# greatscottgadgets/libbtbb

Measured on AMD Instinct MI355X. Metric: Gbit/s raw bitstream scanned (LAP_ANY, err<=2), higher is better.
Workload: dtype u64; 1 GPU; promiscuous LAP_ANY scan, 4 GiB packed single-channel synthetic bitstream per GPU, max_ac_errors=2, sync word every 4096 symbols; symbols_per_gpu=34359738305, hits_per_gpu=6402406, parallelism=time-sharded x1 (btbbx_shard_plan: slices + 63-symbol halo), no collectives

## Files before the change

libbtbb_amd/csrc/context.cpp:

```cpp
#include <stdarg.h>
#include <stdio.h>
#include <stdlib.h>
#include <string.h>
#include <mutex>
#include <shared_mutex>
#include <vector>
#include "common.h"

#define NO_DEVICE_SLOT BTBBX_MAX_DEVICES
static Ctx g_ctx[BTBBX_MAX_DEVICES + 1];
static std::mutex g_init_lock;
static std::shared_mutex g_tables_lock;

void ctx_scan_snapshot(ScanTables *tables, int *table_errors)
{
	std::shared_lock<std::shared_mutex> g(g_tables_lock);
	const Ctx &c = ctx();
	*tables = c.scan;
	*table_errors = c.table_errors;
}
static int g_table_errors = 0;
static thread_local char g_err[512] = "";

static int current_device()
// ... 402 lines not shown
#define BITMAP2_BITS_5 26
static int upload_tables(int max_ac_errors)
{
	const HostTables &t = host_tables();
	Ctx &c = ctx();

	uint64_t entries = 0, binom = 1;
	for (int k = 1; k <= max_ac_errors; k++) {
		binom = binom * (uint64_t)(58 - k + 1) / (uint64_t)k;
		entries += binom;
	}
	int bits = 12;
	while ((1ULL << bits) < 2 * entries + 16)
		bits++;
	while (bits < 20 && (1ULL << bits) < 16 * entries)
		bits++;
	MapBuilder mb;
	mb.slots.assign(1ULL << bits, HSLOT_EMPTY);
	mb.mask = (1ULL << bits) - 1;
	mb.shift = 32 - bits;
	if (max_ac_errors >= 3) {
		const int bits2 = max_ac_errors == 3 ? BITMAP2_BITS_3 : max_ac_errors == 4 ? BITMAP2_BITS_4 : BITMAP2_BITS_5;
		mb.shift2 = 32 - bits2;
		mb.bitmap2.assign(1u << (bits2 - 5), 0);
		mb.bitmap2[0] |= 1u;
	}
	int pos[5];
	for (int k = 1; k <= max_ac_errors; k++)
		mb.enumerate(t, 0, pos, 0, 0, k);

	std::vector<uint32_t> tabA(LDS_TABA_WORDS), tabB(LDS_TABB_WORDS);
	for (uint32_t v = 0; v < LDS_TABA_WORDS; v++) {
		uint64_t s = 0;
		for (int i = 0; i < TABA_BITS; i++)
			if ((v >> i) & 1)
				s ^= t.col[TABA_FIRST + i];
		tabA[v] = (uint32_t)s;
	}
	uint64_t kclass[2];
	kclass[0] = host_syndrome(((uint64_t)BARKER0 << 57) ^ SW_PN);
	kclass[1] = host_syndrome(((uint64_t)BARKER1 << 57) ^ SW_PN);
	for (uint32_t v = 0; v < (1u << TABB_BITS); v++) {
		uint64_t s = kclass[0];
		for (int i = 0; i < TABB_BITS; i++)
			if ((v >> i) & 1)
				s ^= t.col[TABA_FIRST + TABA_BITS + i];
		tabB[v] = (uint32_t)s;
	}

	std::vector<uint32_t> slide_bitmap(SLIDE_WORDS, 0u);
	if (max_ac_errors <= 2) {
		const int rc_slide = build_slide_set(t, max_ac_errors, slide_bitmap);
		if (rc_slide < 0)
			return rc_slide;
		if (slide_bitmap[0] & 3u) {
			set_error("btbbx_init: internal: index 0 / 1 of the sliding checks is a member of the candidate set");
			return BTBBX_E_ARG;
		}
	}

	std::vector<uint32_t> slide4, slide4b;
	if (max_ac_errors == 3 || max_ac_errors == 4) {
		const int rc4 = build_two_level_sets(t, max_ac_errors, slide4, slide4b);
		if (rc4 < 0)
			return rc4;
	} else if (max_ac_errors == 5) {
		const int rc5 = build_five_error_front_set(t, slide4b);
		if (rc5 < 0)
			return rc5;
	}

	size_t off_a = 0, off_b = off_a + 4 * LDS_TABA_WORDS, off_m = off_b + 4 * LDS_TABB_WORDS;
	size_t off_s = off_m;
	size_t off_s4 = off_s + 4 * SLIDE_WORDS, off_s4b = off_s4 + 4 * slide4.size();
	size_t total = off_s4b + 4 * slide4b.size();
	struct Fresh {
		void *tab = nullptr, *hslots = nullptr, *bitmap2 = nullptr;
		~Fresh() { if (tab) (void)hipFree(tab); if (hslots) (void)hipFree(hslots); if (bitmap2) (void)hipFree(bitmap2); }
	} fresh;
	if (!mb.bitmap2.empty()) {
		HIP_TRY(hipMalloc(&fresh.bitmap2, mb.bitmap2.size() * 4));
		HIP_TRY(hipMemcpy(fresh.bitmap2, mb.bitmap2.data(), mb.bitmap2.size() * 4, hipMemcpyHostToDevice));
	}
	HIP_TRY(hipMalloc(&fresh.tab, total));
	HIP_TRY(hipMalloc(&fresh.hslots, mb.slots.size() * sizeof(uint64_t)));
	char *base = (char *)fresh.tab;
	HIP_TRY(hipMemcpy(base + off_a, tabA.data(), 4 * LDS_TABA_WORDS, hipMemcpyHostToDevice));
	HIP_TRY(hipMemcpy(base + off_b, tabB.data(), 4 * LDS_TABB_WORDS, hipMemcpyHostToDevice));
	HIP_TRY(hipMemcpy(base + off_s, slide_bitmap.data(), 4 * SLIDE_WORDS, hipMemcpyHostToDevice));
	if (!slide4.empty())
		HIP_TRY(hipMemcpy(base + off_s4, slide4.data(), 4 * slide4.size(), hipMemcpyHostToDevice));
	if (!slide4b.empty())
		HIP_TRY(hipMemcpy(base + off_s4b, slide4b.data(), 4 * slide4b.size(), hipMemcpyHostToDevice));
	HIP_TRY(hipMemcpy(fresh.hslots, mb.slots.data(), mb.slots.size() * sizeof(uint64_t), hipMemcpyHostToDevice));
	HIP_TRY(hipDeviceSynchronize());
	std::unique_lock<std::shared_mutex> swap_guard(g_tables_lock);
	if (c.d_retired_tab) (void)hipFree(c.d_retired_tab);
	if (c.d_retired_hslots) (void)hipFree(c.d_retired_hslots);
	if (c.d_retired_bitmap2) (void)hipFree(c.d_retired_bitmap2);
	c.d_retired_tab = c.d_tab_block;
	c.d_retired_hslots = c.d_hslots;
	c.d_retired_bitmap2 = c.d_bitmap2;
	c.d_tab_block = fresh.tab;
	c.d_hslots = fresh.hslots;
	c.d_bitmap2 = fresh.bitmap2;
	fresh.tab = fresh.hslots = fresh.bitmap2 = nullptr;
	base = (char *)c.d_tab_block;
	c.scan.tabA = (const uint32_t *)(base + off_a);
	c.scan.tabB = (const uint32_t *)(base + off_b);
	c.scan.slide_bitmap = (const uint32_t *)(base + off_s);
	c.scan.slide4_bitmap = slide4.empty() ? nullptr : (const uint32_t *)(base + off_s4);
	c.scan.slide4b_bitmap = slide4b.empty() ? nullptr : (const uint32_t *)(base + off_s4b);
	c.scan.hslots = (const uint64_t *)c.d_hslots;
	c.scan.hmask = mb.mask;
	c.scan.kclass[0] = kclass[0];
	c.scan.kclass[1] = kclass[1];
	c.scan.kdiff = (uint32_t)(kclass[0] ^ kclass[1]);
	c.scan.hi_mask[0] = c.scan.hi_mask[1] = 0;
	for (int j = 0; j < 57; j++) {
		if ((t.col[j] >> 32) & 1) c.scan.hi_mask[0] |= 1ULL << j;
		if ((t.col[j] >> 33) & 1) c.scan.hi_mask[1] |= 1ULL << j;
	}
	c.scan.bitmap2 = (const uint32_t *)c.d_bitmap2;
	c.scan.bitmap2_shift = (uint32_t)mb.shift2;
	c.table_errors = max_ac_errors;
	return BTBBX_OK;
}

static int init_current_device(int max_ac_errors)
{
	const int dev = current_device();
	if (dev == NO_DEVICE_SLOT) {
		int d = -1;
		(void)hipGetDevice(&d);
		set_error("btbbx_init: HIP device ordinal %d is not below BTBBX_MAX_DEVICES = %d (or hipGetDevice failed)", d,
			  BTBBX_MAX_DEVICES);
		return BTBBX_E_ARG;
	}
	Ctx &c = g_ctx[dev];
	if (g_table_errors == 0 && max_ac_errors > 0)
		g_table_errors = max_ac_errors;
	if (!c.ready) {
		int n = 0;
		hipError_t e = hipGetDeviceCount(&n);
		if (e != hipSuccess || n <= 0) {
			set_error("btbbx_init: no HIP device available (%s) -- this library has no CPU path",
				  e == hipSuccess ? "device count 0" : hipGetErrorString(e));
			return BTBBX_E_NODEVICE;
		}
		c.device = dev;
		hipDeviceProp_t prop;
		HIP_TRY(hipGetDeviceProperties(&prop, dev));
		c.num_cus = prop.multiProcessorCount > 0 ? prop.multiProcessorCount : 256;
		int rc = chain_upload(host_tables());
		if (rc)
			return rc;
		rc = upload_tables(g_table_errors);
		if (rc)
			return rc;
		c.ready = true;
		return BTBBX_OK;
	}
	if (c.table_errors != g_table_errors)
		return upload_tables(g_table_errors);
	return BTBBX_OK;
}
// ... 116 lines not shown
```

libbtbb_amd/csrc/scan_core.h:

```cpp
#pragma once
#include "tile_scan.h"

#define FULL_MASK 0xffffffffffffffffULL

struct ScanArgs {
	const uint64_t *words;
	uint64_t n_words;
	uint64_t pitch_words;
	uint64_t search_bits;
	uint64_t tiles_per_stream;
	uint64_t n_tiles;
	uint32_t xcd_tiles;
	uint32_t ring_margin;
	uint32_t full_tiles;
	uint32_t n_streams;
	uint32_t msb;
	uint32_t lap;
	uint64_t syncword;
	int max_err;
	btbbx_hit *hits;
	uint32_t hit_cap;
	uint32_t *hit_count;
	unsigned long long *first;
	uint32_t *bucket_cnt;
// ... 23 lines not shown
#define PROF_MARK(k) do { (void)(k); } while (0)
#define PROF_PIN(x) do { } while (0)
#endif

__device__ __forceinline__ void count_bucket(const ScanArgs &a, uint32_t stream, uint64_t offset)
{
	if (a.bucket_cnt)
		atomicAdd(&a.bucket_cnt[((uint64_t)stream * a.bucket_mul + offset) >> a.bucket_shift], 1u);
}

__device__ __forceinline__ void emit_hit(const ScanArgs &a, uint32_t stream, uint64_t offset,
					 uint32_t lap, uint32_t nerr)
{
	if (a.first) {
		unsigned long long v = ((unsigned long long)offset << 32) | ((unsigned long long)(lap & 0xffffff) << 8) | nerr;
		atomicMin(a.first, v);
		return;
	}
	uint32_t idx = atomicAdd(a.hit_count, 1u);
	if (idx < a.hit_cap) {
		btbbx_hit h;
		h.offset = offset;
		h.lap = lap;
		h.ac_errors = (uint8_t)nerr;
		h.reserved = 0;
		h.stream = (uint16_t)stream;
		a.hits[idx] = h;
		count_bucket(a, stream, offset);
	}
}

__device__ __forceinline__ uint64_t stream_ld(const uint64_t *p)
{
	return *p;
}
__device__ __forceinline__ uint32_t msb_dword(uint32_t x)
{
	return __builtin_bswap32(__brev(x));
}
__device__ __forceinline__ uint64_t load_word(const uint64_t *base, uint64_t j, uint64_t n_words)
{
	return j < n_words ? stream_ld(base + j) : 0ULL;
}

typedef __attribute__((address_space(3))) uint32_t lds_u32_t;
__device__ __forceinline__ uint32_t lds_ld(uint32_t byte_off) { return *reinterpret_cast<lds_u32_t *>(byte_off); }
__device__ __forceinline__ void lds_st(uint32_t byte_off, uint32_t v) { *reinterpret_cast<lds_u32_t *>(byte_off) = v; }
typedef __attribute__((address_space(3))) uint16_t lds_u16_t;
__device__ __forceinline__ uint32_t lds_ld16(uint32_t byte_off) { return *reinterpret_cast<lds_u16_t *>(byte_off); }
__device__ __forceinline__ uint64_t sign16_after_shl(uint32_t x, uint32_t sh)
{
	uint32_t r;
	uint64_t m;
	asm("v_lshlrev_b16 %1, %2, %3\n\tv_cmp_gt_i16_e64 %0, 0, %1" : "=s"(m), "=&v"(r) : "v"(sh), "v"(x));
	return m;
}
typedef __attribute__((address_space(3))) u32x4 lds_u32x4_t;
__device__ __forceinline__ u32x4 lds_ld4(uint32_t byte_off) { return *reinterpret_cast<lds_u32x4_t *>(byte_off); }
__device__ __forceinline__ void lds_st4(uint32_t byte_off, u32x4 v) { *reinterpret_cast<lds_u32x4_t *>(byte_off) = v; }
__device__ __forceinline__ void lds_st_rec(uint32_t byte_off, u32x4 v)
{
	lds_st(byte_off, v.x);
	lds_st(byte_off + 4u, v.y);
	lds_st(byte_off + 8u, v.z);
	lds_st(byte_off + 12u, v.w);
}
__device__ __forceinline__ void lds_st_rec2(uint32_t byte_off, uint32_t x, uint32_t y, uint32_t z, uint32_t w)
{
	asm volatile("ds_write2_b32 %0, %1, %2 offset1:1\n\tds_write2_b32 %0, %3, %4 offset0:2 offset1:3"
		     : : "v"(byte_off), "v"(x), "v"(y), "v"(z), "v"(w) : "memory");
}

#define SYN3_WORDS 640u
#define SYN3_BYTES (4u * SYN3_WORDS)
static_assert(TABA_FIRST == 34 && TABA_BITS == 11 && TABB_BITS == 12, "the SYN3 tables are cut for window bits 34 .. 56 as 8 + 8 + 7");
__device__ __forceinline__ uint32_t syn3_entry(const ScanTables &t, uint32_t i)
{
	if (i < 256u)
		return t.tabA[i];
	if (i < 512u)
		return t.tabA[((i - 256u) & 7u) << 8] ^ t.tabB[(i - 256u) >> 3] ^ t.tabB[0];
	return t.tabB[(i - 512u) << 5];
}
template <bool LDS_TABLES = true, bool TWO = false>
__device__ __forceinline__ bool verify_lap_any(const ScanArgs &a, uint64_t w, uint32_t &lap, uint32_t &nerr_out, uint32_t syn3_off = 0)
{
	uint32_t win = (uint32_t)(w >> 57);
	uint32_t cls = __popc(win ^ BARKER1) <= 1 ? 1u : 0u;
	uint64_t sw = (w & LOW57) | ((uint64_t)(cls ? BARKER1 : BARKER0) << 57);
	const uint64_t low = w & LOW57;
	const uint32_t ia = (uint32_t)(low >> TABA_FIRST) & ((1u << TABA_BITS) - 1), ib = (uint32_t)(low >> (TABA_FIRST + TABA_BITS));
	uint32_t s_lo;
	if constexpr (TWO) {
		const uint32_t hi = (uint32_t)(low >> 32);
		s_lo = (uint32_t)low ^ lds_ld(syn3_off + (hi & 0x3fcu)) ^ lds_ld(syn3_off + 1024u + ((hi >> 8) & 0x3fcu))
		       ^ lds_ld(syn3_off + 2048u + ((hi >> 16) & 0x1fcu)) ^ (cls ? a.t.kdiff : 0u);
	} else {
		s_lo = (uint32_t)low ^ (LDS_TABLES ? lds_ld(LDS_OFF_TABA + (ia << 2)) : a.t.tabA[ia])
		       ^ (LDS_TABLES ? lds_ld(LDS_OFF_TABB + (ib << 2)) : a.t.tabB[ib]) ^ (cls ? a.t.kdiff : 0u);
	}
	uint32_t s_hi;
	if constexpr (TWO) {
		const uint32_t l0 = (uint32_t)low, l1 = (uint32_t)(low >> 32);
		const uint32_t f0 = (l0 & (uint32_t)a.t.hi_mask[0]) ^ (l1 & (uint32_t)(a.t.hi_mask[0] >> 32));
		const uint32_t f1 = (l0 & (uint32_t)a.t.hi_mask[1]) ^ (l1 & (uint32_t)(a.t.hi_mask[1] >> 32));
		s_hi = ((uint32_t)(a.t.kclass[cls] >> 32) ^ (__popc(f0) & 1) ^ ((__popc(f1) & 1) << 1)) & 3;
	} else {
		s_hi = ((uint32_t)(a.t.kclass[cls] >> 32) ^ (__popcll(low & a.t.hi_mask[0]) & 1)
			^ ((__popcll(low & a.t.hi_mask[1]) & 1) << 1)) & 3;
	}
	const uint64_t syn = ((uint64_t)s_hi << 32) | s_lo;
	if (!TWO && a.t.bitmap2) {
		const uint32_t i2 = (s_lo * 0x9E3779B1u) >> a.t.bitmap2_shift;
		if (!((a.t.bitmap2[i2 >> 5] >> (i2 & 31)) & 1))
			return false;
	}
	uint32_t nerr = 0;
	if (syn) {
		uint64_t h = ((((uint32_t)syn ^ (uint32_t)(syn >> 32)) * 0x9E3779B1u) >> (32 - __popcll(a.t.hmask))) & a.t.hmask;
		for (;;) {
			uint64_t slot = a.t.hslots[h];
			if (slot == HSLOT_EMPTY)
				return false;
			if ((slot & 0x3ffffffffULL) == syn) {
				if constexpr (TWO) {
					const uint32_t p0 = (uint32_t)(slot >> 34) & 63, p1 = (uint32_t)(slot >> 40) & 63;
					sw ^= (1ULL << p0) | (1ULL << p1);
					nerr = p1 != 63 ? 2u : 1u;
					break;
				}
				uint64_t err = 0;
#pragma unroll
				for (int i = 0; i < 5; i++) {
					uint32_t pos = (uint32_t)(slot >> (34 + 6 * i)) & 63;
					if (pos != 63)
						err |= 1ULL << pos;
				}
				sw ^= err;
				nerr = __popcll(err);
				break;
			}
			h = (h + 1) & a.t.hmask;
		}
	}
	lap = (uint32_t)(sw >> 34) & 0xffffff;
	nerr_out = nerr;
	return (int)nerr <= a.max_err;
}


__device__ __forceinline__ void barker32(uint32_t dm, uint32_t dh, uint32_t valid, uint32_t &pass, uint32_t &cls)
{
	const uint32_t s0 = alignbit(dh, dm, 25), s1 = alignbit(dh, dm, 26), s2 = alignbit(dh, dm, 27);
	const uint32_t s3 = alignbit(dh, dm, 28), s4 = alignbit(dh, dm, 29), s5 = alignbit(dh, dm, 30);
	const uint32_t s6 = alignbit(dh, dm, 31);
	const uint32_t a = BITOP3(s0, s1, s2, 0x69);
	const uint32_t ca = BITOP3(s0, s1, s2, 0x17);
	const uint32_t b = BITOP3(s3, s4, s5, 0x69);
	const uint32_t cb = BITOP3(s3, s4, s5, 0xd4);
	const uint32_t cc = BITOP3(a, b, s6, 0xe8);
	pass = BITOP3(ca, cb, cc, 0x81) & valid;
	cls = BITOP3(ca, cb, cc, 0x01);
}

struct Probe { uint32_t x, offA, offB; };

__device__ __forceinline__ Probe probe_addr(uint32_t e0, uint32_t e1, uint32_t e2, uint32_t cls,
					    uint32_t kdiff, uint32_t p)
{
	Probe r;
	const uint32_t wlo = alignbit(e1, e0, p);
	const uint32_t whi = alignbit(e2, e1, p);
	r.offA = whi & (((1u << TABA_BITS) - 1) << 2);
	r.offB = (whi >> (TABA_FIRST - 32 + TABA_BITS - 2)) & (((1u << TABB_BITS) - 1) << 2);
	const uint32_t cmask = (uint32_t)__builtin_amdgcn_sbfe(cls, p, 1);
	r.x = BITOP3(cmask, kdiff, wlo, 0x6a);
	return r;
}

#ifndef PRIO_FILTER
#define PRIO_FILTER 0
#define PRIO_LOOP 2
#define PRIO_CAND 3
#endif
struct SlideTapList { int n; int k[32]; };
template <uint64_t TAPS>
constexpr SlideTapList slide_tap_list()
{
	SlideTapList l = {0, {0}};
	for (int k = 0; k < 64; k++)
		if ((TAPS >> k) & 1)
			l.k[l.n++] = k;
	return l;
}
template <uint64_t TAPS>
__device__ __forceinline__ uint32_t slide32(uint32_t e0, uint32_t e1, uint32_t e2)
{
	constexpr SlideTapList taps = slide_tap_list<TAPS>();
	uint32_t plane[32];
#pragma unroll
	for (int i = 0; i < taps.n; i++) {
		const int k = taps.k[i];
		if (k == 0)
			plane[i] = e0;
		else if (k < 32)
			plane[i] = alignbit(e1, e0, k);
		else if (k == 32)
			plane[i] = e1;
		else
			plane[i] = alignbit(e2, e1, k - 32);
	}
	uint32_t acc = plane[0];
#pragma unroll
	for (int i = 1; i + 1 < taps.n; i += 2)
		acc = xor3(acc, plane[i], plane[i + 1]);
	if ((taps.n & 1) == 0)
		acc ^= plane[taps.n - 1];
	return acc;
}


#define TILE_ORDER(a, first_tile, tile_step, n_mine) \
	uint32_t first_tile = blockIdx.x, tile_step = gridDim.x, n_mine; \
	if (a.xcd_tiles) { \
		const uint32_t xcd = blockIdx.x & 7, lo_t = xcd * a.xcd_tiles; \
		const uint32_t hi_t = min((uint64_t)lo_t + a.xcd_tiles, a.n_tiles); \
		tile_step = gridDim.x >> 3; \
		first_tile = lo_t + (blockIdx.x >> 3); \
		n_mine = first_tile < hi_t ? (hi_t - first_tile + tile_step - 1) / tile_step : 0; \
	} else { \
// ... 63 lines not shown
```

libbtbb_amd/csrc/scan_slide.h:

```cpp
#pragma once
#include "scan_core.h"

#define SLIDE_TILES 2
#define SLIDE4_TILES 3
#define SLIDE_WGS 2
#define SLIDE_THREADS 768
#define SLIDE_FIXED 6
#define SLIDE_DRAIN_AT 60u
#define SLIDE_DRAIN_AT_ORD 40u
struct SlideStd {
	static constexpr int BITS = SLIDE_BITS, THREADS = SLIDE_THREADS, WGS = SLIDE_WGS;
	static constexpr uint64_t TAPS = SLIDE_TAPS, TAPS_B = 0;
	static constexpr bool LEVEL2 = false, INVERT = false, DENSE = false;
	static constexpr bool TWO_ERRORS = true;
};
struct Slide4 {
	static constexpr int BITS = SLIDE4_BITS, THREADS = 1024, WGS = 1;
	static constexpr uint64_t TAPS = SLIDE4_TAPS, TAPS_B = SLIDE4B_TAPS;
	static constexpr bool LEVEL2 = true, INVERT = true, DENSE = true;
	static constexpr bool TWO_ERRORS = false;
};
template <class CFG> struct SlideGeom {
	static constexpr uint32_t SET_WORDS = 1u << (CFG::BITS - 5), SET_BYTES = 4u * SET_WORDS;
	static constexpr uint32_t WAVES_PER_EU = CFG::WGS * CFG::THREADS / 256;
#ifdef SCAN_PROFILE
	static constexpr uint32_t RING = 64;
#else
	static constexpr uint32_t RING = CFG::WGS == 2 ? 64 : 128;
#endif
	static constexpr uint32_t LANE_WORDS = 63;
	static constexpr uint32_t TILE_WORDS = CFG::THREADS / 64 * LANE_WORDS;
	static constexpr uint32_t RING_END = SET_BYTES + CAND_BYTES * (CFG::THREADS / 64) * RING;
	static constexpr uint32_t SYN3_OFF = RING_END;
	static constexpr uint32_t PROF_OFF = SYN3_OFF + (CFG::TWO_ERRORS ? SYN3_BYTES : 0u);
#ifdef SCAN_PROFILE
	static constexpr uint32_t LDS_BYTES = PROF_OFF + 128u * (CFG::THREADS / 64);
#else
	static constexpr uint32_t LDS_BYTES = PROF_OFF;
#endif
	static_assert((uint64_t)LDS_BYTES * CFG::WGS <= 160u * 1024u, "the workgroups a CU is cut for must fit its 160 KiB of LDS");
};

template <class CFG, int TILES, bool MSB, bool ORD = false>
__global__ __launch_bounds__(CFG::THREADS) __attribute__((amdgpu_waves_per_eu(SlideGeom<CFG>::WAVES_PER_EU, SlideGeom<CFG>::WAVES_PER_EU)))
void scan_slide_kernel(ScanArgs a)
{
	extern __shared__ uint32_t lds[];
	if (a.gate && *a.gate == 0)
		return;
	constexpr uint32_t RING = SlideGeom<CFG>::RING;
	constexpr bool ABS = !CFG::LEVEL2;
	constexpr uint32_t THREADS = CFG::THREADS, SET_WORDS = SlideGeom<CFG>::SET_WORDS, SET_BYTES = SlideGeom<CFG>::SET_BYTES;

	const uint32_t tid = threadIdx.x;
	const uint32_t lane = tid & 63;
	const uint32_t wave = __builtin_amdgcn_readfirstlane(tid >> 6);
	constexpr uint32_t LANE_WORDS = SlideGeom<CFG>::LANE_WORDS, TILE_WORDS = SlideGeom<CFG>::TILE_WORDS;
	const uint32_t wid = wave * LANE_WORDS + lane;
	uint32_t live = lane != 63 ? 0xffffffffu : 0u;
	asm volatile("" : "+v"(live));
	const uint32_t ring_off = SET_BYTES + CAND_BYTES * wave * RING;

	TILE_ORDER(a, first_tile, tile_step, n_mine)

	{
		const uint4 *src = reinterpret_cast<const uint4 *>(CFG::LEVEL2 ? a.t.slide4_bitmap : a.t.slide_bitmap);
		uint4 *dst = reinterpret_cast<uint4 *>(lds);
		auto rev16 = [](uint32_t x) { const uint32_t r = __brev(x); return (r >> 16) | (r << 16); };
		for (uint32_t i = tid; i < SET_WORDS / 4; i += THREADS) {
			const uint4 v = src[i];
			dst[i] = make_uint4(rev16(v.x), rev16(v.y), rev16(v.z), rev16(v.w));
		}
	}
	constexpr uint32_t SYN3_OFF = SlideGeom<CFG>::SYN3_OFF;
	if constexpr (CFG::TWO_ERRORS) {
		for (uint32_t i = tid; i < SYN3_WORDS; i += THREADS)
			lds_st(SYN3_OFF + 4u * i, syn3_entry(a.t, i));
	}
	__syncthreads();

#ifdef SCAN_PROFILE
	const uint32_t prof_off = SlideGeom<CFG>::PROF_OFF + 128u * wave;
	if (lane < 32)
		lds_st(prof_off + 4u * lane, 0u);
	uint64_t prof_t;
	asm volatile("s_memtime %0\n\ts_waitcnt lgkmcnt(0)" : "=s"(prof_t) : : "memory");
#endif
	uint32_t q_head = 0, q_tail = 0;
	uint32_t code_tile = 0;
	CODE_WORD_CLOSURE(TILE_WORDS, LANE_WORDS, code_tile = t);
	HIT_QUEUE_CLOSURES();
	auto drain = [&](uint32_t n) {
		bool hit = false;
		uint32_t stream = 0, lap = 0, nerr = 0;
		uint64_t offset = 0;
		u32x4 rec = {0u, 0u, 0u, 0u};
		if (lane < n)
			rec = lds_ld4(ring_off + CAND_BYTES * ((q_head + lane) & (RING - 1)));
		const uint32_t code = rec.x;
		const uint64_t word = code_word(code, stream);
		if (lane < n) {
			const uint64_t w = ((uint64_t)alignbit(rec.w, rec.z, code) << 32) | alignbit(rec.z, rec.y, code);
			offset = word * 64 + (code & 63);
			hit = verify_lap_any<false, CFG::TWO_ERRORS>(a, w, lap, nerr, SYN3_OFF);
		}
		if constexpr (ORD) {
			const uint64_t hm = __ballot(hit);
			if (hm) {
				uint32_t rank = 0, count = 0;
				const uint32_t it_mine = code >> 12;
				const uint32_t it_lo = (uint32_t)__builtin_amdgcn_readfirstlane((int)it_mine) & ~1u;
				const uint32_t it_hi = (uint32_t)__builtin_amdgcn_readlane((int)it_mine, (int)(n - 1)) | 1u;
				bool fast = it_hi - it_lo < 64u;
				if (fast) {
					const uint32_t key = (it_mine - it_lo) & 63u;
					lds_st(ring_off + 4u * lane, 0u);
					uint32_t idx = 0;
					if (hit) {
						idx = __hip_atomic_fetch_add(reinterpret_cast<lds_u32_t *>(ring_off + 4u * key), 1u, __ATOMIC_RELAXED, __HIP_MEMORY_SCOPE_WORKGROUP);
						if (idx < 4u)
							*reinterpret_cast<__attribute__((address_space(3))) uint16_t *>(ring_off + 256u + 8u * key + 2u * idx) = (uint16_t)(code & 0xfffu);
					}
					asm volatile("s_waitcnt lgkmcnt(0)" ::: "memory");
					if (hit)
						count = lds_ld(ring_off + 4u * key);
					if (__ballot(count > 4u)) {
						fast = false;
					} else if (hit) {
						const uint32_t lo2 = lds_ld(ring_off + 256u + 8u * key), hi2 = lds_ld(ring_off + 260u + 8u * key);
						const uint32_t mine = code & 0xfffu;
						rank = ((lo2 & 0xffffu) < mine ? 1u : 0u);
						rank += count > 1u && (lo2 >> 16) < mine ? 1u : 0u;
						rank += count > 2u && (hi2 & 0xffffu) < mine ? 1u : 0u;
						rank += count > 3u && (hi2 >> 16) < mine ? 1u : 0u;
					}
				}
				if (!fast) {
					rank = count = 0;
					for (uint64_t r = hm; r; r &= r - 1) {
						const uint32_t cj = (uint32_t)__builtin_amdgcn_readlane((int)code, (int)__builtin_ctzll(r));
						const bool same = (code ^ cj) < 4096u;
						count += same ? 1u : 0u;
						rank += same && cj < code ? 1u : 0u;
					}
				}
				const uint32_t seg = stream * a.segs_per_stream + code_tile * (THREADS / 64) + wave;
				uint4 out;
				out.x = (uint32_t)offset;
				out.y = (uint32_t)(offset >> 32);
				out.z = lap;
				out.w = nerr | (stream << 16);
				const bool spill = hit && rank >= a.seg_slot_n;
				if (hit && !spill)
					a.seg_slots[(uint64_t)seg * a.seg_slot_n + rank] = (uint64_t)(code & 0xfffu) | ((uint64_t)lap << 12) | ((uint64_t)nerr << 36);
				if (hit && rank + 1 == count)
					a.seg_cnt[seg] = (uint16_t)count;
				const uint64_t om = __ballot(spill);
				if (om) {
					uint32_t base = 0;
					if (lane == 0)
						base = atomicAdd(a.ovf_count, (uint32_t)__popcll(om));
					base = __builtin_amdgcn_readfirstlane(base);
					const uint32_t idx = base + __builtin_amdgcn_mbcnt_hi((uint32_t)(om >> 32), __builtin_amdgcn_mbcnt_lo((uint32_t)om, 0));
					if (spill) {
						if (idx < a.ovf_cap) {
							reinterpret_cast<uint4 *>(a.ovf_recs)[idx] = out;
							a.ovf_meta[idx] = make_uint2(seg, rank);
						} else {
							*a.irregular = 1u;
						}
					}
				}
			}
		} else {
			push_hits(hit, stream, offset, lap, nerr);
		}
		q_head += n;
	};

	struct Cursor { uint32_t stream; uint32_t t; const uint64_t *tp; };
	const uint32_t tiles_per_stream = (uint32_t)a.tiles_per_stream;
	Cursor cur = {a.n_streams, 0, a.words};
	uint32_t handed = 0;
	auto tile_address = [&](const Cursor &c) { return a.words + (uint64_t)c.stream * a.pitch_words + (uint64_t)c.t * TILE_WORDS; };
	if (n_mine) {
		cur.stream = a.n_streams > 1 ? first_tile / tiles_per_stream : 0;
		cur.t = first_tile - cur.stream * tiles_per_stream;
		cur.tp = tile_address(cur);
	}
	auto step_words = [&]() {
		uint32_t ts = tile_step;
		asm volatile("" : "+s"(ts));
		return (uint64_t)ts * TILE_WORDS;
	};
	auto advance = [&](Cursor &c) {
		if (++handed >= n_mine) {
			c.stream = a.n_streams;
			return;
		}
		c.t += tile_step;
		c.tp += step_words();
		if (c.t >= tiles_per_stream) {
			while (c.t >= tiles_per_stream && c.stream < a.n_streams) {
				c.t -= tiles_per_stream;
				c.stream++;
			}
			c.tp = tile_address(c);
		}
	};
	auto tile_full = [&](uint32_t tt) { return tt < a.full_tiles; };
	uint32_t voff = wid * 8u;
	asm volatile("" : "+v"(voff));
	auto load_pair = [&](const Cursor &c, uint64_t &lo, uint64_t &hi) {
		uint32_t bytes = 0;
		if (c.stream < a.n_streams) {
			bytes = (TILE_WORDS + 2u) * 8u;
			if (!tile_full(c.t)) {
				const uint64_t first = (uint64_t)c.t * TILE_WORDS;
				const uint64_t left = first < a.n_words ? a.n_words - first : 0;
				bytes = (uint32_t)(left < TILE_WORDS + 2u ? left : TILE_WORDS + 2u) * 8u;
			}
		}
		const __amdgpu_buffer_rsrc_t rsrc = __builtin_amdgcn_make_buffer_rsrc(const_cast<uint64_t *>(c.tp), 0, (int)bytes, 0x00020000);
		const u32x4 v = __builtin_amdgcn_raw_buffer_load_b128(rsrc, (int)voff, 0, 0);
		lo = ((uint64_t)v.y << 32) | v.x;
		hi = ((uint64_t)v.w << 32) | v.z;
	};

	Cursor tc[TILES];
	uint64_t lo[TILES], hi[TILES];
#pragma unroll
	for (int u = 0; u < TILES; u++) {
		tc[u] = cur;
		load_pair(cur, lo[u], hi[u]);
		advance(cur);
	}

	for (uint32_t it = 0; tc[0].stream < a.n_streams; it += TILES) {
		__builtin_amdgcn_s_setprio(PRIO_FILTER);
		uint32_t d[TILES][4], m[TILES][2], c[TILES][3];
		uint32_t c2[TILES][CFG::LEVEL2 ? 3 : 1];
#pragma unroll
		for (int u = 0; u < TILES; u++) {
			d[u][0] = (uint32_t)lo[u]; d[u][1] = (uint32_t)(lo[u] >> 32);
			d[u][2] = (uint32_t)hi[u]; d[u][3] = (uint32_t)(hi[u] >> 32);
			if constexpr (MSB) {
#pragma unroll
				for (int k = 0; k < 4; k++)
					d[u][k] = msb_dword(d[u][k]);
			}
			uint32_t cls_unused;
			barker32(d[u][1], d[u][2], live, m[u][0], cls_unused);
			barker32(d[u][2], d[u][3], live, m[u][1], cls_unused);
			if (tc[u].stream >= a.n_streams) {
				m[u][0] = m[u][1] = 0;
			} else if (!tile_full(tc[u].t)) {
				const uint64_t first_off = ((uint64_t)tc[u].t * TILE_WORDS + wid) * 64;
				const uint64_t valid = first_off >= a.search_bits ? 0ULL
					: (a.search_bits - first_off >= 64 ? FULL_MASK : ((1ULL << (a.search_bits - first_off)) - 1));
				m[u][0] &= (uint32_t)valid;
				m[u][1] &= (uint32_t)(valid >> 32);
			}
			c[u][0] = slide32<CFG::TAPS>(d[u][0], d[u][1], d[u][2]);
			c[u][1] = slide32<CFG::TAPS>(d[u][1], d[u][2], d[u][3]);
			if constexpr (CFG::INVERT) {
				c[u][0] = ~c[u][0];
				c[u][1] = ~c[u][1];
			}
			c[u][2] = (uint32_t)__builtin_amdgcn_ds_bpermute((int)((lane + 1) << 2), (int)c[u][0]);
			if constexpr (CFG::LEVEL2) {
				c2[u][0] = slide32<CFG::TAPS_B>(d[u][0], d[u][1], d[u][2]);
				c2[u][1] = slide32<CFG::TAPS_B>(d[u][1], d[u][2], d[u][3]);
				c2[u][2] = (uint32_t)__builtin_amdgcn_ds_bpermute((int)((lane + 1) << 2), (int)c2[u][0]);
			}
		}

		uint64_t C[TILES][2];
#pragma unroll
		for (int u = 0; u < TILES; u++)
#pragma unroll
			for (int h = 0; h < 2; h++)
				C[u][h] = ((uint64_t)(ABS ? c[u][h + 1] : (c[u][h + 1] | 0x80000000u)) << 32) | c[u][h];
		struct Stage { uint32_t v[TILES][2], bw[TILES][2]; };
		auto any_left = [&]() {
			uint32_t any = 0;
#pragma unroll
			for (int u = 0; u < TILES; u++)
				any |= m[u][0] | m[u][1];
			return __ballot(any != 0) != 0;
		};
		uint32_t pos2[TILES][2];
		auto event_chain = [&](int u, int h, uint64_t cm) {
			const bool cand = __builtin_amdgcn_inverse_ballot_w64(cm);
			const uint32_t room = RING - (q_tail - q_head);
			uint32_t in_wave;
			asm("s_bcnt1_i32_b64 %0, %1" : "=s"(in_wave) : "s"(cm) : "scc");
			const uint32_t n = min(in_wave, room);
			if (cand) {
				uint32_t lane6 = lane << 6;
				asm volatile("" : "+v"(lane6));
				uint32_t pos;
				if constexpr (ABS)
					pos = pos2[u][h];
				else if constexpr (CFG::LEVEL2)
					pos = pos2[u][h];
				else
					asm("v_ffbh_u32 %0, %1" : "=v"(pos) : "v"((uint32_t)(C[u][h] >> 32)));
				const uint32_t code = pos | lane6 | (((it + u) << 12) | (h << 5));
				const u32x4 rec = {code, d[u][h], d[u][h + 1], d[u][h + 2]};
				if (in_wave == 1 && room) {
					lds_st_rec(ring_off + CAND_BYTES * (q_tail & (RING - 1)), rec);
				} else {
					const uint32_t rank = __builtin_amdgcn_mbcnt_hi((uint32_t)(cm >> 32),
							__builtin_amdgcn_mbcnt_lo((uint32_t)cm, 0));
					if (rank < room) {
						lds_st_rec(ring_off + CAND_BYTES * ((q_tail + rank) & (RING - 1)), rec);
					} else {
						uint32_t stream, lap, nerr, cold = code;
						asm volatile("" : "+v"(cold));
						const uint64_t word = code_word(cold, stream);
						const uint32_t wlo = alignbit(rec.z, rec.y, pos), whi = alignbit(rec.w, rec.z, pos);
// ... 132 lines not shown
		auto level2_take = [&]() {
			if (!any_sent)
				return;
			uint64_t cms[TILES][2], any = 0;
#pragma unroll
			for (int u = 0; u < TILES; u++)
#pragma unroll
				for (int h = 0; h < 2; h++) {
					cms[u][h] = sent[u][h] & __ballot((int32_t)(w2[u][h] << (v2[u][h] & 31)) < 0);
					any |= cms[u][h];
				}
			any_sent = 0;
			if (any)
				events(cms);
		};
		auto pass = [&]() {
			Stage g;
#pragma unroll
			for (int u = 0; u < TILES; u++)
#pragma unroll
				for (int h = 0; h < 2; h++)
					step(u, h, g);
			__builtin_amdgcn_sched_barrier(0);
			uint64_t cms[TILES][2], any = 0;
#pragma unroll
			for (int u = 0; u < TILES; u++)
#pragma unroll
				for (int h = 0; h < 2; h++) {
					cms[u][h] = member(u, h, g);
					any |= cms[u][h];
				}
			if constexpr (CFG::LEVEL2) {
				level2_take();
				static_assert(!CFG::LEVEL2 || TILES == 3, "the scalar OR below is written for six chains");
				uint64_t any2;
				asm("s_or_b64 %0, %1, %2\n\ts_or_b64 %0, %0, %3\n\ts_or_b64 %0, %0, %4\n\ts_or_b64 %0, %0, %5\n\ts_or_b64 %0, %0, %6"
				    : "=&s"(any2) : "s"(cms[0][0]), "s"(cms[0][1]), "s"(cms[1][0]), "s"(cms[1][1]), "s"(cms[TILES - 1][0]), "s"(cms[TILES - 1][1]) : "scc");
				if (any2)
					level2_send(cms);
			} else if (any) {
				note_events(cms);
			}
		};
		auto sparse_tail = [&]() {
			uint64_t live[TILES][2], anyl = 0;

#pragma unroll
			for (int u = 0; u < TILES; u++)
#pragma unroll
				for (int h = 0; h < 2; h++) {
					live[u][h] = __ballot(m[u][h] != 0);
					anyl |= live[u][h];
				}
			while (anyl) {
				Stage g;
				uint64_t cms[TILES][2], anyc = 0;
				anyl = 0;
#pragma unroll
				for (int u = 0; u < TILES; u++)
#pragma unroll
					for (int h = 0; h < 2; h++) {
						cms[u][h] = 0;
						if (!live[u][h])
							continue;
						step(u, h, g);
						cms[u][h] = member(u, h, g);
						anyc |= cms[u][h];
						live[u][h] = __ballot(m[u][h] != 0);
						anyl |= live[u][h];
					}
				if (anyc)
					note_events(cms);
			}
		};
#ifdef SCAN_PROFILE
#pragma unroll
		for (int u = 0; u < TILES; u++) {
			PROF_PIN(m[u][0]); PROF_PIN(m[u][1]); PROF_PIN(c[u][0]); PROF_PIN(c[u][1]); PROF_PIN(c[u][2]);
		}
#endif
		PROF_MARK(0);
		uint32_t pass_no = 1;
		if constexpr (!CFG::DENSE) {
			__builtin_amdgcn_s_setprio(PRIO_LOOP);
#pragma unroll 1
			for (int k = 0; k < SLIDE_FIXED; k++) {
				pass();
				PROF_MARK(pass_no < 13 ? pass_no : 13);
				pass_no++;
			}
			sparse_tail();
			append_noted();
			PROF_MARK(pass_no < 13 ? pass_no : 13);
			__builtin_amdgcn_s_setprio(PRIO_CAND);
			PROF_MARK(16);
			if (q_tail - q_head >= (RING == 64 ? (ORD ? SLIDE_DRAIN_AT_ORD : SLIDE_DRAIN_AT) : 64u))
				drain(q_tail - q_head > 64 ? 64 : q_tail - q_head);
		} else {
			for (;;) {
				__builtin_amdgcn_s_setprio(PRIO_LOOP);
				bool more = true;
				while (q_tail - q_head + a.ring_margin <= RING) {
					if (!any_left()) {
						more = false;
						break;
					}
					pass();
					PROF_MARK(pass_no < 13 ? pass_no : 13);
					pass_no++;
				}
				if constexpr (CFG::LEVEL2)
					level2_take();
				__builtin_amdgcn_s_setprio(PRIO_CAND);
				PROF_MARK(16);
				if (more || q_tail - q_head >= 32u)
					drain(q_tail - q_head > 64 ? 64 : q_tail - q_head);
				if (!more)
					break;
			}
		}
		(void)pass_no;
		PROF_MARK(18);
#pragma unroll
		for (int u = 0; u < TILES; u++) {
			tc[u] = cur;
			load_pair(cur, lo[u], hi[u]);
			advance(cur);
		}
		PROF_MARK(19);
	}
	while (q_tail != q_head)
		drain(q_tail - q_head > 64 ? 64 : q_tail - q_head);
	flush_hits();
#ifdef SCAN_PROFILE
	if (lane < 32)
		atomicAdd(&g_scan_prof[lane], (unsigned long long)lds_ld(prof_off + 4u * lane));
#endif
}
```

Baseline: 13290 Gbit/s.

## Split slide drain into issue and deferred verify to hide hash-slot latency

The sparse slide path's candidate drain is split in two. The first half computes syndromes and issues the global hash-slot load, fetching two adjacent slots as one vector load. The second half finishes probing and pushes hits at the top of the next tile iteration, so the global load latency overlaps with tile loads and filtering. A duplicated sentinel slot is appended to the table so the paired load stays in bounds. The cost is extra live registers across the loop and added code-path complexity.

```diff
diff --git a/libbtbb_amd/csrc/context.cpp b/libbtbb_amd/csrc/context.cpp
--- a/libbtbb_amd/csrc/context.cpp
+++ b/libbtbb_amd/csrc/context.cpp
@@ -508,6 +508,7 @@
 		HIP_TRY(hipMalloc(&fresh.bitmap2, mb.bitmap2.size() * 4));
 		HIP_TRY(hipMemcpy(fresh.bitmap2, mb.bitmap2.data(), mb.bitmap2.size() * 4, hipMemcpyHostToDevice));
 	}
+	mb.slots.push_back(mb.slots[0]);
 	HIP_TRY(hipMalloc(&fresh.tab, total));
 	HIP_TRY(hipMalloc(&fresh.hslots, mb.slots.size() * sizeof(uint64_t)));
 	char *base = (char *)fresh.tab;
diff --git a/libbtbb_amd/csrc/scan_core.h b/libbtbb_amd/csrc/scan_core.h
--- a/libbtbb_amd/csrc/scan_core.h
+++ b/libbtbb_amd/csrc/scan_core.h
@@ -129,70 +129,104 @@
 		return t.tabA[((i - 256u) & 7u) << 8] ^ t.tabB[(i - 256u) >> 3] ^ t.tabB[0];
 	return t.tabB[(i - 512u) << 5];
 }
+__device__ __forceinline__ uint64_t lap_syndrome2(const ScanArgs &a, uint64_t w, uint64_t &sw, uint32_t syn3_off)
+{
+	const uint32_t win = (uint32_t)(w >> 57);
+	const uint32_t cls = __popc(win ^ BARKER1) <= 1 ? 1u : 0u;
+	sw = (w & LOW57) | ((uint64_t)(cls ? BARKER1 : BARKER0) << 57);
+	const uint64_t low = w & LOW57;
+	const uint32_t hi = (uint32_t)(low >> 32);
+	const uint32_t s_lo = (uint32_t)low ^ lds_ld(syn3_off + (hi & 0x3fcu)) ^ lds_ld(syn3_off + 1024u + ((hi >> 8) & 0x3fcu))
+			      ^ lds_ld(syn3_off + 2048u + ((hi >> 16) & 0x1fcu)) ^ (cls ? a.t.kdiff : 0u);
+	const uint32_t l0 = (uint32_t)low, l1 = (uint32_t)(low >> 32);
+	const uint32_t f0 = (l0 & (uint32_t)a.t.hi_mask[0]) ^ (l1 & (uint32_t)(a.t.hi_mask[0] >> 32));
+	const uint32_t f1 = (l0 & (uint32_t)a.t.hi_mask[1]) ^ (l1 & (uint32_t)(a.t.hi_mask[1] >> 32));
+	const uint32_t s_hi = ((uint32_t)(a.t.kclass[cls] >> 32) ^ (__popc(f0) & 1) ^ ((__popc(f1) & 1) << 1)) & 3;
+	return ((uint64_t)s_hi << 32) | s_lo;
+}
+__device__ __forceinline__ uint64_t hslot_of(const ScanTables &t, uint64_t syn)
+{
+	return ((((uint32_t)syn ^ (uint32_t)(syn >> 32)) * 0x9E3779B1u) >> (32 - __popcll(t.hmask))) & t.hmask;
+}
+__device__ __forceinline__ bool hslot_matches(uint64_t slot, uint64_t syn)
+{
+	return (slot & 0x3ffffffffULL) == syn;
+}
+__device__ __forceinline__ uint32_t slot_errors2(uint64_t slot, uint64_t &sw)
+{
+	const uint32_t p0 = (uint32_t)(slot >> 34) & 63, p1 = (uint32_t)(slot >> 40) & 63;
+	sw ^= (1ULL << p0) | (1ULL << p1);
+	return p1 != 63 ? 2u : 1u;
+}
+__device__ __forceinline__ uint32_t lap_of(uint64_t sw)
+{
+	return (uint32_t)(sw >> 34) & 0xffffff;
+}
 template <bool LDS_TABLES = true, bool TWO = false>
 __device__ __forceinline__ bool verify_lap_any(const ScanArgs &a, uint64_t w, uint32_t &lap, uint32_t &nerr_out, uint32_t syn3_off = 0)
 {
-	uint32_t win = (uint32_t)(w >> 57);
-	uint32_t cls = __popc(win ^ BARKER1) <= 1 ? 1u : 0u;
-	uint64_t sw = (w & LOW57) | ((uint64_t)(cls ? BARKER1 : BARKER0) << 57);
-	const uint64_t low = w & LOW57;
-	const uint32_t ia = (uint32_t)(low >> TABA_FIRST) & ((1u << TABA_BITS) - 1), ib = (uint32_t)(low >> (TABA_FIRST + TABA_BITS));
-	uint32_t s_lo;
 	if constexpr (TWO) {
-		const uint32_t hi = (uint32_t)(low >> 32);
-		s_lo = (uint32_t)low ^ lds_ld(syn3_off + (hi & 0x3fcu)) ^ lds_ld(syn3_off + 1024u + ((hi >> 8) & 0x3fcu))
-		       ^ lds_ld(syn3_off + 2048u + ((hi >> 16) & 0x1fcu)) ^ (cls ? a.t.kdiff : 0u);
-	} else {
-		s_lo = (uint32_t)low ^ (LDS_TABLES ? lds_ld(LDS_OFF_TABA + (ia << 2)) : a.t.tabA[ia])
-		       ^ (LDS_TABLES ? lds_ld(LDS_OFF_TABB + (ib << 2)) : a.t.tabB[ib]) ^ (cls ? a.t.kdiff : 0u);
-	}
-	uint32_t s_hi;
-	if constexpr (TWO) {
-		const uint32_t l0 = (uint32_t)low, l1 = (uint32_t)(low >> 32);
-		const uint32_t f0 = (l0 & (uint32_t)a.t.hi_mask[0]) ^ (l1 & (uint32_t)(a.t.hi_mask[0] >> 32));
-		const uint32_t f1 = (l0 & (uint32_t)a.t.hi_mask[1]) ^ (l1 & (uint32_t)(a.t.hi_mask[1] >> 32));
-		s_hi = ((uint32_t)(a.t.kclass[cls] >> 32) ^ (__popc(f0) & 1) ^ ((__popc(f1) & 1) << 1)) & 3;
-	} else {
-		s_hi = ((uint32_t)(a.t.kclass[cls] >> 32) ^ (__popcll(low & a.t.hi_mask[0]) & 1)
-			^ ((__popcll(low & a.t.hi_mask[1]) & 1) << 1)) & 3;
-	}
-	const uint64_t syn = ((uint64_t)s_hi << 32) | s_lo;
-	if (!TWO && a.t.bitmap2) {
-		const uint32_t i2 = (s_lo * 0x9E3779B1u) >> a.t.bitmap2_shift;
-		if (!((a.t.bitmap2[i2 >> 5] >> (i2 & 31)) & 1))
-			return false;
-	}
-	uint32_t nerr = 0;
-	if (syn) {
-		uint64_t h = ((((uint32_t)syn ^ (uint32_t)(syn >> 32)) * 0x9E3779B1u) >> (32 - __popcll(a.t.hmask))) & a.t.hmask;
-		for (;;) {
-			uint64_t slot = a.t.hslots[h];
-			if (slot == HSLOT_EMPTY)
-				return false;
-			if ((slot & 0x3ffffffffULL) == syn) {
-				if constexpr (TWO) {
-					const uint32_t p0 = (uint32_t)(slot >> 34) & 63, p1 = (uint32_t)(slot >> 40) & 63;
-					sw ^= (1ULL << p0) | (1ULL << p1);
-					nerr = p1 != 63 ? 2u : 1u;
+		uint64_t sw;
+		const uint64_t syn = lap_syndrome2(a, w, sw, syn3_off);
+		uint32_t nerr = 0;
+		if (syn) {
+			uint64_t h = hslot_of(a.t, syn);
+			for (;;) {
+				const uint64_t slot = a.t.hslots[h];
+				if (slot == HSLOT_EMPTY)
+					return false;
+				if (hslot_matches(slot, syn)) {
+					nerr = slot_errors2(slot, sw);
 					break;
 				}
-				uint64_t err = 0;
+				h = (h + 1) & a.t.hmask;
+			}
+		}
+		lap = lap_of(sw);
+		nerr_out = nerr;
+		return (int)nerr <= a.max_err;
+	} else {
+		uint32_t win = (uint32_t)(w >> 57);
+		uint32_t cls = __popc(win ^ BARKER1) <= 1 ? 1u : 0u;
+		uint64_t sw = (w & LOW57) | ((uint64_t)(cls ? BARKER1 : BARKER0) << 57);
+		const uint64_t low = w & LOW57;
+		const uint32_t ia = (uint32_t)(low >> TABA_FIRST) & ((1u << TABA_BITS) - 1), ib = (uint32_t)(low >> (TABA_FIRST + TABA_BITS));
+		const uint32_t s_lo = (uint32_t)low ^ (LDS_TABLES ? lds_ld(LDS_OFF_TABA + (ia << 2)) : a.t.tabA[ia])
+				      ^ (LDS_TABLES ? lds_ld(LDS_OFF_TABB + (ib << 2)) : a.t.tabB[ib]) ^ (cls ? a.t.kdiff : 0u);
+		const uint32_t s_hi = ((uint32_t)(a.t.kclass[cls] >> 32) ^ (__popcll(low & a.t.hi_mask[0]) & 1)
+				       ^ ((__popcll(low & a.t.hi_mask[1]) & 1) << 1)) & 3;
+		const uint64_t syn = ((uint64_t)s_hi << 32) | s_lo;
+		if (a.t.bitmap2) {
+			const uint32_t i2 = (s_lo * 0x9E3779B1u) >> a.t.bitmap2_shift;
+			if (!((a.t.bitmap2[i2 >> 5] >> (i2 & 31)) & 1))
+				return false;
+		}
+		uint32_t nerr = 0;
+		if (syn) {
+			uint64_t h = ((((uint32_t)syn ^ (uint32_t)(syn >> 32)) * 0x9E3779B1u) >> (32 - __popcll(a.t.hmask))) & a.t.hmask;
+			for (;;) {
+				uint64_t slot = a.t.hslots[h];
+				if (slot == HSLOT_EMPTY)
+					return false;
+				if ((slot & 0x3ffffffffULL) == syn) {
+					uint64_t err = 0;
 #pragma unroll
-				for (int i = 0; i < 5; i++) {
-					uint32_t pos = (uint32_t)(slot >> (34 + 6 * i)) & 63;
-					if (pos != 63)
-						err |= 1ULL << pos;
+					for (int i = 0; i < 5; i++) {
+						uint32_t pos = (uint32_t)(slot >> (34 + 6 * i)) & 63;
+						if (pos != 63)
+							err |= 1ULL << pos;
+					}
+					sw ^= err;
+					nerr = __popcll(err);
+					break;
 				}
-				sw ^= err;
-				nerr = __popcll(err);
-				break;
+				h = (h + 1) & a.t.hmask;
 			}
-			h = (h + 1) & a.t.hmask;
 		}
-	}
-	lap = (uint32_t)(sw >> 34) & 0xffffff;
-	nerr_out = nerr;
-	return (int)nerr <= a.max_err;
+		lap = (uint32_t)(sw >> 34) & 0xffffff;
+		nerr_out = nerr;
+		return (int)nerr <= a.max_err;
+	}
 }
 
 
diff --git a/libbtbb_amd/csrc/scan_slide.h b/libbtbb_amd/csrc/scan_slide.h
--- a/libbtbb_amd/csrc/scan_slide.h
+++ b/libbtbb_amd/csrc/scan_slide.h
@@ -1,4 +1,5 @@
 #pragma once
+#include <type_traits>
 #include "scan_core.h"
 
 #define SLIDE_TILES 2
@@ -8,6 +9,12 @@
 #define SLIDE_FIXED 6
 #define SLIDE_DRAIN_AT 60u
 #define SLIDE_DRAIN_AT_ORD 40u
+#ifndef SLIDE_SPLIT_AT
+#define SLIDE_SPLIT_AT 0
+#endif
+#ifndef SLIDE_SPLIT_SLOTS
+#define SLIDE_SPLIT_SLOTS 2
+#endif
 struct SlideStd {
 	static constexpr int BITS = SLIDE_BITS, THREADS = SLIDE_THREADS, WGS = SLIDE_WGS;
 	static constexpr uint64_t TAPS = SLIDE_TAPS, TAPS_B = 0;
@@ -90,19 +97,81 @@
 	uint32_t code_tile = 0;
 	CODE_WORD_CLOSURE(TILE_WORDS, LANE_WORDS, code_tile = t);
 	HIT_QUEUE_CLOSURES();
-	auto drain = [&](uint32_t n) {
+	static_assert(SLIDE_SPLIT_AT >= 0 && SLIDE_SPLIT_AT <= 2, "head, behind the filter, or end of the trip");
+	constexpr bool SPLIT = !CFG::DENSE && !(ORD && SLIDE_SPLIT_AT == 2);
+	static_assert(!SPLIT || CFG::TWO_ERRORS, "the split drain has no test of a second-level bitmap");
+	uint32_t p_n = 0;
+	uint32_t p_code = 0, p_swhi = 0, p_synlo = 0, p_synhi = 0;
+	uint64_t p_slot = 0, p_slot2 = 0;
+	auto drain_issue = [&](uint32_t n) {
+		u32x4 rec = {0u, 0u, 0u, 0u};
+		if (lane < n)
+			rec = lds_ld4(ring_off + CAND_BYTES * ((q_head + lane) & (RING - 1)));
+		p_code = rec.x;
+		const uint64_t w = ((uint64_t)alignbit(rec.w, rec.z, p_code) << 32) | alignbit(rec.z, rec.y, p_code);
+		uint64_t sw;
+		const uint64_t syn = lap_syndrome2(a, w, sw, SYN3_OFF);
+#if SLIDE_SPLIT_SLOTS == 2
+		{
+			typedef uint64_t slot_pair_t __attribute__((ext_vector_type(2), aligned(8)));
+			const slot_pair_t two = *reinterpret_cast<const slot_pair_t *>(a.t.hslots + hslot_of(a.t, syn));
+			p_slot = two.x;
+			p_slot2 = two.y;
+		}
+#else
+		p_slot = a.t.hslots[hslot_of(a.t, syn)];
+#endif
+		p_swhi = (uint32_t)(sw >> 32);
+		p_synlo = (uint32_t)syn;
+		p_synhi = (uint32_t)(syn >> 32);
+		p_n = n;
+		q_head += n;
+	};
+	const std::false_type whole;
+	const std::true_type second_half;
+	auto drain = [&](uint32_t n, auto half) {
+		constexpr bool SECOND = decltype(half)::value;
 		bool hit = false;
 		uint32_t stream = 0, lap = 0, nerr = 0;
 		uint64_t offset = 0;
 		u32x4 rec = {0u, 0u, 0u, 0u};
-		if (lane < n)
+		if constexpr (SECOND)
+			rec.x = p_code;
+		else if (lane < n)
 			rec = lds_ld4(ring_off + CAND_BYTES * ((q_head + lane) & (RING - 1)));
 		const uint32_t code = rec.x;
 		const uint64_t word = code_word(code, stream);
 		if (lane < n) {
-			const uint64_t w = ((uint64_t)alignbit(rec.w, rec.z, code) << 32) | alignbit(rec.z, rec.y, code);
-			offset = word * 64 + (code & 63);
-			hit = verify_lap_any<false, CFG::TWO_ERRORS>(a, w, lap, nerr, SYN3_OFF);
+			if constexpr (SECOND) {
+				offset = word * 64 + (code & 63);
+				const uint64_t syn = ((uint64_t)p_synhi << 32) | p_synlo;
+				uint64_t sw = (uint64_t)p_swhi << 32;
+				bool found = true;
+				if (syn) {
+					uint64_t slot = p_slot;
+#if SLIDE_SPLIT_SLOTS == 2
+					if (slot != HSLOT_EMPTY && !hslot_matches(slot, syn))
+						slot = p_slot2;
+#endif
+					if (slot != HSLOT_EMPTY && !hslot_matches(slot, syn)) {
+						uint64_t h = hslot_of(a.t, syn) + (SLIDE_SPLIT_SLOTS - 1);
+						do {
+							h = (h + 1) & a.t.hmask;
+							slot = a.t.hslots[h];
+						} while (slot != HSLOT_EMPTY && !hslot_matches(slot, syn));
+					}
+					if (slot == HSLOT_EMPTY)
+						found = false;
+					else
+						nerr = slot_errors2(slot, sw);
+				}
+				lap = lap_of(sw);
+				hit = found && (int)nerr <= a.max_err;
+			} else {
+				const uint64_t w = ((uint64_t)alignbit(rec.w, rec.z, code) << 32) | alignbit(rec.z, rec.y, code);
+				offset = word * 64 + (code & 63);
+				hit = verify_lap_any<false, CFG::TWO_ERRORS>(a, w, lap, nerr, SYN3_OFF);
+			}
 		}
 		if constexpr (ORD) {
 			const uint64_t hm = __ballot(hit);
@@ -175,7 +244,10 @@
 		} else {
 			push_hits(hit, stream, offset, lap, nerr);
 		}
-		q_head += n;
+		if constexpr (SECOND)
+			p_n = 0;
+		else
+			q_head += n;
 	};
 
 	struct Cursor { uint32_t stream; uint32_t t; const uint64_t *tp; };
@@ -237,6 +309,10 @@
 	}
 
 	for (uint32_t it = 0; tc[0].stream < a.n_streams; it += TILES) {
+		if constexpr (SPLIT && SLIDE_SPLIT_AT == 0) {
+			if (p_n)
+				drain(p_n, second_half);
+		}
 		__builtin_amdgcn_s_setprio(PRIO_FILTER);
 		uint32_t d[TILES][4], m[TILES][2], c[TILES][3];
 		uint32_t c2[TILES][CFG::LEVEL2 ? 3 : 1];
@@ -535,6 +611,12 @@
 		PROF_MARK(0);
 		uint32_t pass_no = 1;
 		if constexpr (!CFG::DENSE) {
+			if constexpr (SPLIT && SLIDE_SPLIT_AT == 1) {
+				if (p_n) {
+					__builtin_amdgcn_s_setprio(PRIO_CAND);
+					drain(p_n, second_half);
+				}
+			}
 			__builtin_amdgcn_s_setprio(PRIO_LOOP);
 #pragma unroll 1
 			for (int k = 0; k < SLIDE_FIXED; k++) {
@@ -543,12 +625,22 @@
 				pass_no++;
 			}
 			sparse_tail();
+			if constexpr (SPLIT && SLIDE_SPLIT_AT == 2) {
+				if (p_n) {
+					__builtin_amdgcn_s_setprio(PRIO_CAND);
+					drain(p_n, second_half);
+				}
+			}
 			append_noted();
 			PROF_MARK(pass_no < 13 ? pass_no : 13);
 			__builtin_amdgcn_s_setprio(PRIO_CAND);
 			PROF_MARK(16);
-			if (q_tail - q_head >= (RING == 64 ? (ORD ? SLIDE_DRAIN_AT_ORD : SLIDE_DRAIN_AT) : 64u))
-				drain(q_tail - q_head > 64 ? 64 : q_tail - q_head);
+			if (q_tail - q_head >= (RING == 64 ? (ORD ? SLIDE_DRAIN_AT_ORD : SLIDE_DRAIN_AT) : 64u)) {
+				if constexpr (SPLIT)
+					drain_issue(q_tail - q_head > 64 ? 64 : q_tail - q_head);
+				else
+					drain(q_tail - q_head > 64 ? 64 : q_tail - q_head, whole);
+			}
 		} else {
 			for (;;) {
 				__builtin_amdgcn_s_setprio(PRIO_LOOP);
@@ -567,7 +659,7 @@
 				__builtin_amdgcn_s_setprio(PRIO_CAND);
 				PROF_MARK(16);
 				if (more || q_tail - q_head >= 32u)
-					drain(q_tail - q_head > 64 ? 64 : q_tail - q_head);
+					drain(q_tail - q_head > 64 ? 64 : q_tail - q_head, whole);
 				if (!more)
 					break;
 			}
@@ -582,8 +674,18 @@
 		}
 		PROF_MARK(19);
 	}
-	while (q_tail != q_head)
-		drain(q_tail - q_head > 64 ? 64 : q_tail - q_head);
+	if constexpr (SPLIT) {
+		for (;;) {
+			if (p_n)
+				drain(p_n, second_half);
+			if (q_tail == q_head)
+				break;
+			drain_issue(q_tail - q_head > 64 ? 64 : q_tail - q_head);
+		}
+	} else {
+		while (q_tail != q_head)
+			drain(q_tail - q_head > 64 ? 64 : q_tail - q_head, whole);
+	}
 	flush_hits();
 #ifdef SCAN_PROFILE
 	if (lane < 32)
```

Measured after the change: 13480 Gbit/s, median of 6. +1.5%, better.
